# gabrieletiboni/random-envs

Hardware: AMD Instinct MI355X
Metric: env-steps/sec at batch 32768, RandomHopper-v0, 1/2/4/8 MI355X; % HBM roofline (higher is better)
Workload: dtype f32

## Files before the change

profiles/wavetime_probe.py:

```python
import os, sys, ctypes
os.environ.setdefault("REX_LIB", "librex_hip_wavetime.so")
sys.path.insert(0, os.path.dirname(os.path.dirname(os.path.abspath(__file__))))
import numpy as np, torch, random_envs_amd as rex
from random_envs_amd import _native
for eid in sys.argv[1:] or ["RandomHopper-v0"]:
    B = 32768
    env = rex.make(eid, batch=B, seed=0)
    nom = torch.tensor(env.original_task)
    env.set_dr_distribution("uniform", torch.stack([0.9 * nom, 1.1 * nom], 1).flatten().tolist()); env.set_dr_training(True); env.reset()
    g = torch.Generator().manual_seed(0)
    amp = 0.4 if "Humanoid" in eid else 1.0
    acts = [((torch.rand(env.dims.act_dim, B, generator=g) * 2 - 1) * amp).cuda() for _ in range(8)]
    for k in range(80 if "Humanoid" in eid else 300): env.step_soa(acts[k % 8])
    rows, infos = [], []
    info = (ctypes.c_ulonglong * (1024 * 8))(); torch.cuda.synchronize(); _native.lib().rex_debug_waveinfo(info, 1024)
    for k in range(20):
        env.step_soa(acts[k % 8]); torch.cuda.synchronize()
        out = (ctypes.c_ulonglong * 1024)(); _native.lib().rex_debug_wavetime(out, 1024)
        _native.lib().rex_debug_waveinfo(info, 1024)
        rows.append(np.array(list(out), dtype=np.float64)); infos.append(np.array(list(info), dtype=np.float64).reshape(1024, 8))
    w = np.stack(rows); I = np.stack(infos)
    if hasattr(_native.lib(), "rex_debug_wavephase") and "Humanoid" not in eid:
        ph = (ctypes.c_ulonglong * (1024 * 4))(); _native.lib().rex_debug_wavephase(ph, 1024)
        P = np.array(list(ph), dtype=np.float64).reshape(1024, 4)
        env.enable_timing(True); env.step_soa(acts[0]); torch.cuda.synchronize(); ms = env.read_timing()[-1]; env.enable_timing(False)
        print("   last launch, cycles per wave [mean / max]: load state %.0f / %.0f | substeps %.0f / %.0f | reward, obs, stores %.0f / %.0f | fused reset %.0f / %.0f | "
              "sum of means %.0f, slowest wave %.0f; kernel %.4f ms" % (P[:, 0].mean(), P[:, 0].max(), P[:, 1].mean(), P[:, 1].max(), P[:, 2].mean(), P[:, 2].max(),
                                                                     P[:, 3].mean(), P[:, 3].max(), P.sum(1).mean(), P.sum(1).max(), ms))
    if hasattr(_native.lib(), "rex_debug_evalphase") and "Humanoid" not in eid:
        ep = (ctypes.c_ulonglong * (1024 * 16))(); _native.lib().rex_debug_evalphase(ep, 1024)
        for k in range(10): env.step_soa(acts[k % 8])
        torch.cuda.synchronize(); _native.lib().rex_debug_evalphase(ep, 1024)
        E = np.array(list(ep), dtype=np.float64).reshape(1024, 16).mean(0) / 10
        nm = ["kinematics", "mass+bias+forces", "detect", "self / a0 / dispatch", "rows + solve", "  pass 1 (all)", "  pass 2 (all)"]
        print("   cycles per wave-step by phase of forward() (16 evaluations): " + " | ".join("%s %.0f" % (nm[k], E[k]) for k in range(7)) + " | sum of 0..4 %.0f" % E[:5].sum())
    print(eid, "cycles per wave-step: mean %.0f  p50 %.0f  p90 %.0f  p99 %.0f  max %.0f  -> max/mean %.2f" %
          (w.mean(), np.percentile(w, 50), np.percentile(w, 90), np.percentile(w, 99), w.max(1).mean(), w.max(1).mean() / w.mean()))
    print("   cycles in the fused reset path per wave-step: mean %.0f  p90 %.0f  max %.0f" % (I[..., 1].mean(), np.percentile(I[..., 1], 90), I[..., 1].max(1).mean()))
    print("   the same wave slow twice in a row (rank correlation of consecutive launches): %.2f" % np.corrcoef(w[:-1].ravel(), w[1:].ravel())[0, 1])
    names = ["solves", "reset cycles", "pass1", "pass2", "ls_evals", "nocon", "slots_active", "selfpath"]
    slow = w > np.percentile(w, 98); fast = w < np.percentile(w, 60)
    print("   per wave-step counts, typical waves (< p60) vs slow waves (> p98):")
    top = w.argmax(1)
    for k, nm in enumerate(names): print("     %-13s %8.1f %8.1f   slowest wave of each launch: mean %8.1f  min %8.1f  max %8.1f" %
                                         (nm, I[..., k][fast].mean(), I[..., k][slow].mean(), I[np.arange(len(top)), top, k].mean(), I[np.arange(len(top)), top, k].min(), I[np.arange(len(top)), top, k].max()))
    print("   per wave-step counts, mean over ALL waves: " + "  ".join("%s %.2f" % (nm, I[..., k].mean()) for k, nm in enumerate(names)))
    srt = np.sort(w, 1)
    print("   per launch: slowest wave %.0f, 2nd %.0f, 5th %.0f, 10th %.0f, 20th %.0f, 50th %.0f cycles (means over the launches)" %
          tuple(srt[:, -k].mean() for k in (1, 2, 5, 10, 20, 50)))
    env.close()
```

random-envs_amd/csrc/rex_hip.hip:

```cpp
#include <hip/hip_runtime.h>
#include <rocrand/rocrand_kernel.h>

#include <cmath>
#include <cstdarg>
#include <cstdio>
#include <cstdlib>
#include <cstring>
#include <new>
#include <vector>

#include "../../include/rex.h"
#include "planar_model.hpp"
#include "humanoid_model.hpp"
#include "humanoid_pair.hpp"

using namespace rex;

#ifdef REX_ONLY_KIND
#define REX_EN_CARTPOLE (REX_ONLY_KIND == 0)
#define REX_EN_HOPPER (REX_ONLY_KIND == 1)
#define REX_EN_HALFCHEETAH (REX_ONLY_KIND == 2)
#define REX_EN_WALKER2D (REX_ONLY_KIND == 3)
#define REX_EN_HUMANOID (REX_ONLY_KIND == 4)
#else
#define REX_EN_CARTPOLE 1
#define REX_EN_HOPPER 1
#define REX_EN_HALFCHEETAH 1
#define REX_EN_WALKER2D 1
#define REX_EN_HUMANOID 1
#endif

#if defined(REX_KTIME)
namespace rex { __device__ unsigned long long g_ktime[24 + 72]; }
extern "C" int rex_debug_ktime(unsigned long long* out) {
  if (hipMemcpyFromSymbol(out, HIP_SYMBOL(rex::g_ktime), sizeof(unsigned long long) * 96) != hipSuccess) return -1;
  unsigned long long z[96] = {0}; (void)hipMemcpyToSymbol(HIP_SYMBOL(rex::g_ktime), z, sizeof z); return 0; }
#endif
#if defined(REX_WAVETIME)
namespace rex { __device__ unsigned long long g_wavetime[8192]; __device__ unsigned long long g_waveinfo[8192][8]; __device__ unsigned long long g_wavehum[1024][16];
                __device__ unsigned long long g_wavephase[8192][4];
                __device__ unsigned long long g_waveplace[8192][4];
                }
#endif
#if defined(REX_WAVETIME) || defined(REX_PHASES)
namespace rex { __device__ unsigned long long g_evalphase[8192][16]; }
extern "C" int rex_debug_evalphase(unsigned long long* out, int n) {
  if (hipMemcpyFromSymbol(out, HIP_SYMBOL(rex::g_evalphase), sizeof(unsigned long long) * 16 * (n < 8192 ? n : 8192)) != hipSuccess) return -1;
  static unsigned long long z[8192][16]; return hipMemcpyToSymbol(HIP_SYMBOL(rex::g_evalphase), z, sizeof z) == hipSuccess ? 0 : -1; }
#endif
#if defined(REX_WAVETIME)
extern "C" int rex_debug_wavephase(unsigned long long* out, int n) {
  return hipMemcpyFromSymbol(out, HIP_SYMBOL(rex::g_wavephase), sizeof(unsigned long long) * 4 * (n < 8192 ? n : 8192)) == hipSuccess ? 0 : -1; }
extern "C" int rex_debug_waveplace(unsigned long long* out, int n) {
  return hipMemcpyFromSymbol(out, HIP_SYMBOL(rex::g_waveplace), sizeof(unsigned long long) * 4 * (n < 8192 ? n : 8192)) == hipSuccess ? 0 : -1; }
extern "C" int rex_debug_wavehum(unsigned long long* out) {
  return hipMemcpyFromSymbol(out, HIP_SYMBOL(rex::g_wavehum), sizeof(unsigned long long) * 1024 * 16) == hipSuccess ? 0 : -1; }
extern "C" int rex_debug_waveinfo(unsigned long long* out, int n) {
  if (hipMemcpyFromSymbol(out, HIP_SYMBOL(rex::g_waveinfo), sizeof(unsigned long long) * 8 * (n < 8192 ? n : 8192)) != hipSuccess) return -1;
  static unsigned long long z[8192][8]; return hipMemcpyToSymbol(HIP_SYMBOL(rex::g_waveinfo), z, sizeof z) == hipSuccess ? 0 : -1; }
extern "C" int rex_debug_wavetime(unsigned long long* out, int n) {
  return hipMemcpyFromSymbol(out, HIP_SYMBOL(rex::g_wavetime), sizeof(unsigned long long) * (n < 8192 ? n : 8192)) == hipSuccess ? 0 : -1; }
#endif
#if defined(REX_KSTATS)
namespace rex { __device__ unsigned long long g_kstats[8]; }
extern "C" int rex_debug_kstats(unsigned long long* out) {
  if (hipMemcpyFromSymbol(out, HIP_SYMBOL(rex::g_kstats), sizeof(unsigned long long) * 8) != hipSuccess) return -1;
  unsigned long long z[8] = {0}; (void)hipMemcpyToSymbol(HIP_SYMBOL(rex::g_kstats), z, sizeof z); return 0; }
#endif

static thread_local char g_err[512] = "";
static int set_err(int code, const char* fmt, ...) {
  va_list ap; va_start(ap, fmt); vsnprintf(g_err, sizeof g_err, fmt, ap); va_end(ap);
  return code;
}
#define HIP_TRY(x)                                                                            \
  do { hipError_t e_ = (x); if (e_ != hipSuccess) return set_err(REX_ERR_HIP, "%s failed: %s", #x, hipGetErrorString(e_)); } while (0)

extern "C" const char* rex_last_error(void) { return g_err; }
extern "C" const char* rex_version(void) { return "rex-hip 0.1 (gfx950)"; }

#define REX_ENTER(h, fn)                                                    \
  do { if (!(h)) return set_err(REX_ERR_ARG, fn ": null handle"); HIP_TRY(hipSetDevice((h)->device)); } while (0)

static const char* const kKnobs[] = {"REX_LANES", "REX_PAIR", "REX_ROLLED", "REX_HUM_PAIR", "REX_HUM_FUSED_RESET", "REX_FUSED_DERIVE",
                                     "REX_FAST", "REX_LS_MAX", "REX_LS_FREE", "REX_WARM", "REX_CORR",
                                     "REX_DIAG_NOCONTACT", "REX_HUM_ITERS"};
static bool tuning_allowed() { const char* e = getenv("REX_ALLOW_TUNING"); return e && atoi(e) == 1; }
static const char* stray_knob() {
  if (tuning_allowed()) return nullptr;
  for (const char* k : kKnobs) if (getenv(k)) return k;
  return nullptr;
}
static const char* knob(const char* name) { return tuning_allowed() ? getenv(name) : nullptr; }

constexpr int MAX_XI = 32;
struct DRParams {
  int type;
  int dim;
  float a[MAX_XI];
  float b[MAX_XI];
  float lower[MAX_XI];
  float lo[MAX_XI], hi[MAX_XI];
  int map[MAX_XI];
  const float* chol;
};

constexpr unsigned long long EP_STRIDE = 1ull << 32;
constexpr unsigned long long STEP_BASE = 512, STEP_STRIDE = 64;
constexpr unsigned long long SAMPLE_SEED_SALT = 0x9E3779B97F4A7C15ull;

__device__ __forceinline__ float truncnorm2(float u) {
  const float Fa = 0.022750131948179195f, Fb = 0.9772498680518208f;
  float p = Fa + u * (Fb - Fa);
  float x = normcdfinvf(p);
  return fminf(fmaxf(x, -2.0f), 2.0f);
}

__device__ void sample_task(const DRParams& dr, unsigned long long seed, unsigned long long subseq, unsigned long long offset,
                            float* __restrict__ xi_rows, size_t B, unsigned i, unsigned long long* counters) {
  const int d = dr.dim;
  rocrand_state_philox4x32_10 st;
  rocrand_init(seed, subseq, offset, &st);
  if (dr.type == REX_DR_UNIFORM) {
    for (int k = 0; k < d; k++) { float u = rocrand_uniform(&st); (xi_rows + (size_t)dr.map[k] * B)[i] = dr.a[k] + (dr.b[k] - dr.a[k]) * (1.0f - u); }
  } else if (dr.type == REX_DR_TRUNCNORM) {
    for (int k = 0; k < d; k++) {
      float lb = dr.lower[k];
      float obs = dr.a[k] + dr.b[k] * truncnorm2(rocrand_uniform(&st));
      for (int att = 0; att < 2 && obs < lb; att++) obs = dr.a[k] + dr.b[k] * truncnorm2(rocrand_uniform(&st));
      if (obs < lb) obs = lb;
      (xi_rows + (size_t)dr.map[k] * B)[i] = obs;
    }
  } else if (dr.type == REX_DR_GAUSSIAN) {
    for (int k = 0; k < d; k++) {
      float obs = dr.a[k] + dr.b[k] * rocrand_normal(&st);
      for (int att = 0; att < 2 && obs < 0.1f; att++) obs = dr.a[k] + dr.b[k] * rocrand_normal(&st);
      if (obs < 0.1f) { obs = 0.1f; atomicAdd(counters + 1, 1ull); }
      (xi_rows + (size_t)dr.map[k] * B)[i] = obs;
    }
  } else if (dr.type == REX_DR_FULLGAUSSIAN) {
    for (int k = 0; k < d; k++) {
      rocrand_state_philox4x32_10 sz; rocrand_init(seed, subseq, offset, &sz);
      float acc = dr.a[k];
      for (int j = 0; j <= k; j++) acc += dr.chol[k * MAX_XI + j] * rocrand_normal(&sz);
      acc = fminf(fmaxf(acc, 0.0f), 4.0f);
      (xi_rows + (size_t)dr.map[k] * B)[i] = acc * (dr.hi[k] - dr.lo[k]) * 0.25f + dr.lo[k];
    }
  }
}

struct DevState {
  float* qpos; float* qvel; float* xi;
  float* geom;
  float* aux;
  int* t; unsigned* episode; unsigned char* done;
  unsigned long long* counters;
  long long B, env_offset;
  unsigned long long seed;
};

struct StepFlags {
  int endless, noisy, time_limit, max_steps;
  float noise_std;
  float* info;
  int readonly;
};

__global__ void __launch_bounds__(64) cartpole_step_kernel(DevState s, StepFlags fl, const int* __restrict__ action,
                                                           float* __restrict__ obs, float* __restrict__ reward,
                                                           unsigned char* __restrict__ done_out, unsigned char* __restrict__ trunc_out,
                                                           float* __restrict__ term_obs) {
  const unsigned i = blockIdx.x * blockDim.x + threadIdx.x;
  if (i >= s.B) return;
  const long long B = s.B;
  float x = s.qpos[i], th = s.qpos[B + i], xd = s.qvel[i], thd = s.qvel[B + i];
  float g = s.xi[i], mc = s.xi[B + i], mp = s.xi[2 * B + i], l = s.xi[3 * B + i];
  float total = mp + mc;
  const float pml = 0.1f * 0.5f;
  float force = action[i] == 1 ? 10.0f : -10.0f;
  float st, ct; sincosf(th, &st, &ct);
  float temp = (force + pml * thd * thd * st) / total;
  float thacc = (g * st - ct * temp) / (l * (4.0f / 3.0f - mp * ct * ct / total));
  float xacc = temp - pml * thacc * ct / total;
  const float tau = 0.02f;
  x = x + tau * xd; xd = xd + tau * xacc; th = th + tau * thd; thd = thd + tau * thacc;
  s.qpos[i] = x; s.qpos[B + i] = th; s.qvel[i] = xd; s.qvel[B + i] = thd;
  const float th_thr = 12.0f * 2.0f * 3.14159265358979323846f / 360.0f, x_thr = 2.4f;
  bool was_done = s.done[i] != 0;
  bool dn = (x < -x_thr) || (x > x_thr) || (th < -th_thr) || (th > th_thr);
  float r = (!dn) ? 1.0f : (was_done ? 0.0f : 1.0f);
  int t = s.t[i] + 1; s.t[i] = t;
  bool trunc = fl.time_limit && t >= fl.max_steps && !dn;
  bool d = dn || trunc;
  s.done[i] = (unsigned char)((dn || was_done) ? 1 : 0) | (unsigned char)(d ? 2 : 0);
  obs[i] = x; obs[B + i] = xd; obs[2 * B + i] = th; obs[3 * B + i] = thd;
  if (term_obs) { term_obs[i] = x; term_obs[B + i] = xd; term_obs[2 * B + i] = th; term_obs[3 * B + i] = thd; }
  reward[i] = r; done_out[i] = d ? 1 : 0;
  if (trunc_out) trunc_out[i] = trunc ? 1 : 0;
}

__global__ void __launch_bounds__(64) cartpole_reset_kernel(DevState s, DRParams dr, int resample, int reset_state,
                                                            const unsigned char* __restrict__ mask, int mask_bit,
                                                            float* __restrict__ obs) {
  const unsigned i = blockIdx.x * blockDim.x + threadIdx.x;
  if (i >= s.B) return;
  if (mask && !(mask[i] & mask_bit)) return;
  const long long B = s.B;
  unsigned ep = s.episode[i] + 1; s.episode[i] = ep;
  rocrand_state_philox4x32_10 st;
  rocrand_init(s.seed, (unsigned long long)(s.env_offset + i), (unsigned long long)ep * EP_STRIDE, &st);
  if (reset_state) {
    float v[4];
#pragma unroll
    for (int k = 0; k < 4; k++) v[k] = -0.05f + 0.1f * (1.0f - rocrand_uniform(&st));
    s.qpos[i] = v[0]; s.qvel[i] = v[1]; s.qpos[B + i] = v[2]; s.qvel[B + i] = v[3];
    s.t[i] = 0; s.done[i] = 0;
    if (obs) { obs[i] = v[0]; obs[B + i] = v[1]; obs[2 * B + i] = v[2]; obs[3 * B + i] = v[3]; }
  }
  if (resample && dr.type != REX_DR_NONE) {
    sample_task(dr, s.seed, (unsigned long long)(s.env_offset + i), (unsigned long long)ep * EP_STRIDE + 256, s.xi, (size_t)B, i, s.counters);
  }
}

template <class S> constexpr int geom_floats() { return sizeof(PlanarGeom<float, S>) / sizeof(float); }

template <class S>
__device__ __forceinline__ void load_geom(const DevState& s, unsigned i, const PlanarGeom<float, S>& uniform,
                                          PlanarGeom<float, S>& G) {
  if constexpr (S::KIND == 3) {
    walker_expand(uniform, [&](int k) { return (s.geom + (size_t)k * s.B)[i]; }, G);
  } else {
    G = uniform;
  }
}

template <class S>
__device__ __forceinline__ void write_obs(const float (&q)[S::NV], const float (&v)[S::NV], float* __restrict__ obs,
                                          long long B, unsigned i, bool noisy, float noise_std,
                                          rocrand_state_philox4x32_10* st) {
  static_for<0, S::NOBS>([&](auto KK) {
    constexpr int k = KK;
    float o = k < S::NV - 1 ? q[k + 1] : v[k - (S::NV - 1)];
    if (noisy) o += noise_std * rocrand_normal(st);
    (obs + (size_t)k * B)[i] = o;
  });
}

template <class S>
__device__ __forceinline__ void planar_reset_lane(const DevState& s, const StepFlags& fl, const DRParams& dr, int resample,
                                                  int reset_state, unsigned i, float* __restrict__ obs);
__device__ __forceinline__ void walker_derive_lane(const DevState& s, unsigned i, int refresh_frozen_masses);
__device__ __attribute__((noinline)) void walker_derive_call(const DevState& s, unsigned i, int refresh_frozen_masses);
constexpr int RS_RESAMPLE = 1, RS_DERIVE = 2, RS_REFRESH = 4;

#ifndef REX_STEP_WAVES
#define REX_STEP_WAVES 1
#endif
#define REX_STEP_OCC __attribute__((amdgpu_waves_per_eu(REX_STEP_WAVES, REX_STEP_WAVES)))

template <class S, bool PAIR, bool ROLLED = false>
__global__ void __launch_bounds__(64) __attribute__((amdgpu_waves_per_eu(ROLLED ? 2 : REX_STEP_WAVES, ROLLED ? 2 : REX_STEP_WAVES)))
planar_step_kernel(DevState s, StepFlags fl, PlanarGeom<float, S> ugeom,
                                                         SolParams<float> sp, const float* __restrict__ action,
                                                         float* __restrict__ obs, float* __restrict__ reward,
                                                         unsigned char* __restrict__ done_out,
                                                         unsigned char* __restrict__ trunc_out, float* __restrict__ term_obs,
                                                         DRParams dr, int fused_reset, int resample) {
#if defined(REX_WAVETIME)
  const unsigned long long tp0 = __builtin_amdgcn_s_memtime();
  const unsigned long long tw0 = __builtin_amdgcn_s_memrealtime();
#endif
  unsigned blk = blockIdx.x;
  if constexpr (PAIR) { if (blockDim.x < 64u && (gridDim.x & 7u) == 0u) blk = (blk & 7u) * (gridDim.x >> 3) + (blk >> 3); }
  const unsigned i = (blk * blockDim.x + threadIdx.x) >> (PAIR ? 1 : 0);
  if (i >= s.B) return;
  const long long B = s.B;
  float q[S::NV], v[S::NV], ctrl[S::NU], xi[S::NXI];
  static_for<0, S::NV>([&](auto KK) { constexpr int k = KK; q[k] = (s.qpos + (size_t)k * B)[i]; v[k] = (s.qvel + (size_t)k * B)[i]; });
  static_for<0, S::NU>([&](auto KK) { constexpr int k = KK; ctrl[k] = (action + (size_t)k * B)[i]; });
  static_for<0, S::NXI>([&](auto KK) { constexpr int k = KK; xi[k] = (s.xi + (size_t)k * B)[i]; });
  PlanarGeom<float, S> G; load_geom<S>(s, i, ugeom, G);
  LaneParams<float, S> P; lane_params(S{}, xi, P);
#if defined(REX_KTIME) || defined(REX_WAVETIME)
  unsigned long long tk0 = __builtin_amdgcn_s_memtime();
#endif
  const float x_before = q[0];
  q[0] = 0.0f;
  bool capped = false;
  float acc[S::NV];
  static_for<0, S::NV>([&](auto KK) { acc[KK] = 0.0f; });
  constexpr int GEN = PAIR ? 2 : (ROLLED ? 1 : 0);
  float* slot_col = nullptr;
  if constexpr (GEN == 2) {
    __shared__ float slot_lds[SlotMem<float, S, PAIR>::WORDS];
    slot_col = slot_lds + threadIdx.x;
  }
#pragma unroll 1
  for (int f = 0; f < S::FRAME_SKIP; f++) capped |= substep<float, S, PAIR, GEN>(q, v, ctrl, G, P, sp, acc, f > 0, slot_col);
  if (PAIR && (threadIdx.x & 1u)) return;
  unsigned io = i; asm volatile("" : "+v"(io));
#if defined(REX_KTIME)
  if ((threadIdx.x & 63) == 0) atomicAdd(&g_ktime[5], __builtin_amdgcn_s_memtime() - tk0);
#endif
#if defined(REX_WAVETIME)
  const unsigned long long tk1 = __builtin_amdgcn_s_memtime();
  if ((threadIdx.x & 63) == 0) g_wavetime[blockIdx.x & 8191] = tk1 - tk0;
#endif
  const float dx = q[0];
  q[0] = x_before + dx;
  float asq = 0.0f;
  static_for<0, S::NU>([&](auto KK) { asq += ctrl[KK] * ctrl[KK]; });
  const float dt = float(S::TIMESTEP * S::FRAME_SKIP);
  float r = dx / dt + S::ALIVE - S::CTRL_COST * asq;
  bool finite = true;
  static_for<0, S::NV>([&](auto KK) { constexpr int k = KK; finite = finite && isfinite(q[k]) && isfinite(v[k]); });
  bool dn = false;
  if constexpr (S::KIND == 1) {
    bool small = true;
    static_for<2, S::NV>([&](auto KK) { constexpr int k = KK; small = small && fabsf(q[k]) < 100.0f; });
    static_for<0, S::NV>([&](auto KK) { constexpr int k = KK; small = small && fabsf(v[k]) < 100.0f; });
    dn = !(finite && small && q[1] > 0.7f && fabsf(q[2]) < 0.2f);
  } else if constexpr (S::KIND == 3) {
    dn = !(q[1] > 0.8f && q[1] < 2.0f && q[2] > -1.0f && q[2] < 1.0f);
  } else {
    dn = false;
  }
  if (fl.endless) dn = false;
  if (!fl.readonly) {
    if (!finite) atomicAdd(s.counters + 0, 1ull);
    if (capped && threadIdx.x == 0) atomicAdd(s.counters + 2, 1ull);
  }
  int t = s.t[io] + 1;
  bool trunc = fl.time_limit && t >= fl.max_steps && !dn && !fl.readonly;
  bool d = dn || trunc;
  if (!fl.readonly) {
    s.t[io] = t;
    static_for<0, S::NV>([&](auto KK) { constexpr int k = KK; (s.qpos + (size_t)k * B)[io] = q[k]; (s.qvel + (size_t)k * B)[io] = v[k]; });
    s.done[io] = d ? 2 : 0;
  }
  rocrand_state_philox4x32_10 st;
  if (fl.noisy) rocrand_init(s.seed, (unsigned long long)(s.env_offset + io),
                             (unsigned long long)s.episode[io] * EP_STRIDE + STEP_BASE + (unsigned long long)t * STEP_STRIDE, &st);
  write_obs<S>(q, v, obs, B, io, fl.noisy != 0, fl.noise_std, &st);
  if (term_obs) static_for<0, S::NOBS>([&](auto KK) { constexpr int k = KK; (term_obs + (size_t)k * B)[io] = (obs + (size_t)k * B)[io]; });
  reward[io] = r; done_out[io] = d ? 1 : 0;
  if (trunc_out) trunc_out[io] = trunc ? 1 : 0;
  if (fl.info) { fl.info[io] = dx / dt; (fl.info + (size_t)B)[io] = -S::CTRL_COST * asq; }
#if defined(REX_WAVETIME)
  const unsigned long long tr0 = __builtin_amdgcn_s_memtime();
#endif
  if (fused_reset && d) {
    planar_reset_lane<S>(s, fl, dr, resample & RS_RESAMPLE, 1, io, obs);
    if constexpr (S::KIND == 3) {
      if (resample & RS_DERIVE) {
        if constexpr (PAIR) walker_derive_lane(s, io, (resample & RS_REFRESH) ? 1 : 0);
        else walker_derive_call(s, io, (resample & RS_REFRESH) ? 1 : 0);
      }
    }
  }
#if defined(REX_WAVETIME)
  if ((threadIdx.x & 63) == 0) { g_waveinfo[blockIdx.x & 8191][1] += __builtin_amdgcn_s_memtime() - tr0; }
  if ((threadIdx.x & 63) == 0) { unsigned long long* ph = g_wavephase[blockIdx.x & 8191]; ph[0] = tk0 - tp0; ph[1] = tk1 - tk0; ph[2] = tr0 - tk1; ph[3] = __builtin_amdgcn_s_memtime() - tr0; }
  if ((threadIdx.x & 63) == 0) { unsigned long long* pl = g_waveplace[blockIdx.x & 8191]; pl[0] = tw0; pl[1] = __builtin_amdgcn_s_memrealtime();
    pl[2] = __builtin_amdgcn_s_getreg((31 << 11) | (0 << 6) | 4); pl[3] = __builtin_amdgcn_s_getreg((3 << 11) | (0 << 6) | 20); }
#endif
}

template <class S>
__device__ __forceinline__ void planar_reset_lane(const DevState& s, const StepFlags& fl, const DRParams& dr, int resample,
                                                  int reset_state, unsigned i, float* __restrict__ obs) {
  const long long B = s.B;
  unsigned ep = s.episode[i] + 1; s.episode[i] = ep;
#if defined(REX_DIAG_CHEAP_RESET)
  if (reset_state) {
    static_for<0, S::NV>([&](auto KK) { constexpr int k = KK; (s.qpos + (size_t)k * B)[i] = (k == 1 && S::KIND != 2) ? 1.25f : 0.0f; (s.qvel + (size_t)k * B)[i] = 0.0f; });
    s.t[i] = 0; s.done[i] = 0;
  }
  return;
#endif
  if (reset_state) {
    rocrand_state_philox4x32_10 st;
    rocrand_init(s.seed, (unsigned long long)(s.env_offset + i), (unsigned long long)ep * EP_STRIDE, &st);
    float q[S::NV], v[S::NV];
    const float c = S::INIT_NOISE;
    static_for<0, S::NV>([&](auto KK) { constexpr int k = KK;
      q[k] = c * (2.0f * (1.0f - rocrand_uniform(&st)) - 1.0f);
      if constexpr (S::KIND == 2) v[k] = 0.1f * rocrand_normal(&st);
      else v[k] = c * (2.0f * (1.0f - rocrand_uniform(&st)) - 1.0f);
    });
    if constexpr (S::KIND != 2) q[1] += 1.25f;
    static_for<0, S::NV>([&](auto KK) { constexpr int k = KK; (s.qpos + (size_t)k * B)[i] = q[k]; (s.qvel + (size_t)k * B)[i] = v[k]; });
    s.t[i] = 0; s.done[i] = 0;
    if (obs) {
      rocrand_state_philox4x32_10 st2;
      if (fl.noisy) rocrand_init(s.seed, (unsigned long long)(s.env_offset + i), (unsigned long long)ep * EP_STRIDE + STEP_BASE, &st2);
      write_obs<S>(q, v, obs, B, i, fl.noisy != 0, fl.noise_std, &st2);
    }
  }
  if (resample && dr.type != REX_DR_NONE) {
    sample_task(dr, s.seed, (unsigned long long)(s.env_offset + i), (unsigned long long)ep * EP_STRIDE + 256, s.xi, (size_t)B, i, s.counters);
  }
}

template <class S>
__global__ void __launch_bounds__(64) planar_reset_kernel(DevState s, StepFlags fl, DRParams dr, int resample, int reset_state,
                                                          const unsigned char* __restrict__ mask, int mask_bit,
                                                          float* __restrict__ obs, int pending_bit) {
  const unsigned i = blockIdx.x * blockDim.x + threadIdx.x;
  if (i >= s.B) return;
  if (mask && !(mask[i] & mask_bit)) return;
  planar_reset_lane<S>(s, fl, dr, resample, reset_state, i, obs);
  if (pending_bit) s.done[i] = (unsigned char)pending_bit;
}

#if REX_EN_WALKER2D
__global__ void __launch_bounds__(64) walker_derive_kernel(DevState s, const unsigned char* mask, int mask_bit,
                                                           int refresh_frozen_masses, int clear_pending) {
  using S = Walker2dSpec;
  const unsigned i = blockIdx.x * blockDim.x + threadIdx.x;
  if (i >= s.B) return;
  if (mask && !(mask[i] & mask_bit)) return;
  if (clear_pending) s.done[i] = 0;
  walker_derive_lane(s, i, refresh_frozen_masses);
}
__device__ __forceinline__ void walker_derive_lane(const DevState& s, unsigned i, int refresh_frozen_masses) {
  using S = Walker2dSpec;
  double size[4];
  for (int k = 0; k < 4; k++) size[k] = (double)s.xi[(long long)(7 + k) * s.B + i];
  PlanarGeom<double, S> G; SolParams<double> sp; double nominal[S::NB];
  derive_model<double, S>(size, G, nominal, sp);
  double c[kWalkerCompact];
  walker_compact_from_geom(G, c);
  for (int k = 0; k < kWalkerCompact; k++) (s.geom + (size_t)k * s.B)[i] = (float)c[k];
  if (refresh_frozen_masses) for (int b = 0; b < 3; b++) (s.xi + (size_t)b * s.B)[i] = (float)nominal[b];
}
__device__ __attribute__((noinline)) void walker_derive_call(const DevState& s, unsigned i, int refresh_frozen_masses) { walker_derive_lane(s, i, refresh_frozen_masses); }
#else
__device__ __forceinline__ void walker_derive_lane(const DevState&, unsigned, int) {}
__device__ __forceinline__ void walker_derive_call(const DevState&, unsigned, int) {}

#endif

template <class S>
__global__ void __launch_bounds__(64) planar_obs_kernel(DevState s, float* __restrict__ obs) {
  const unsigned i = blockIdx.x * blockDim.x + threadIdx.x;
  if (i >= s.B) return;
  float q[S::NV], v[S::NV];
  static_for<0, S::NV>([&](auto KK) { constexpr int k = KK; q[k] = (s.qpos + (size_t)k * s.B)[i]; v[k] = (s.qvel + (size_t)k * s.B)[i]; });
  write_obs<S>(q, v, obs, s.B, i, false, 0.0f, nullptr);
}
__global__ void __launch_bounds__(64) cartpole_obs_kernel(DevState s, float* __restrict__ obs) {
  const unsigned i = blockIdx.x * blockDim.x + threadIdx.x;
  if (i >= s.B) return;
  const long long B = s.B;
  obs[i] = s.qpos[i]; obs[B + i] = s.qvel[i]; obs[2 * B + i] = s.qpos[B + i]; obs[3 * B + i] = s.qvel[B + i];
}
__global__ void fill_rows_kernel(float* dst, const float* vals, int nrows, long long B) {
  long long i = (long long)blockIdx.x * blockDim.x + threadIdx.x;
  if (i >= B) return;
  for (int k = 0; k < nrows; k++) dst[(long long)k * B + i] = vals[k];
}

#if REX_EN_HUMANOID
__constant__ hum::Model<float> c_hum;

__device__ __forceinline__ void hum_lane(const DevState& s, unsigned i, hum::Lane<float>& L) {
  L.mass[0] = 0.0f;
  for (int k = 0; k < 13; k++) L.mass[1 + k] = (s.xi + (size_t)k * s.B)[i];
  for (int d = 0; d < 6; d++) L.damping[d] = 0.0f;
  for (int k = 0; k < 17; k++) L.damping[6 + k] = (s.xi + (size_t)(13 + k) * s.B)[i];
}

__global__ void __launch_bounds__(64) humanoid_step_kernel(DevState s, StepFlags fl, const float* __restrict__ action,
                                                           float* __restrict__ obs, float* __restrict__ reward,
                                                           unsigned char* __restrict__ done_out, unsigned char* __restrict__ trunc_out,
                                                           float* __restrict__ term_obs) {
  const unsigned i = blockIdx.x * blockDim.x + threadIdx.x;
  if (i >= s.B) return;
  const size_t B = (size_t)s.B;
  hum::Lane<float> L; hum_lane(s, i, L);
  float q[hum::NQ], v[hum::NV], a[hum::NU], xp[hum::NBODY];
  for (int k = 0; k < hum::NQ; k++) q[k] = (s.qpos + k * B)[i];
  for (int k = 0; k < hum::NV; k++) v[k] = (s.qvel + k * B)[i];
  for (int k = 0; k < hum::NU; k++) a[k] = (action + k * B)[i];
  for (int b = 0; b < hum::NBODY; b++) xp[b] = (s.aux + b * B)[i];
  hum::Kin<float> kn; hum::Scratch<float> sc;
#if defined(REX_KTIME)
  for (int k = 0; k < HT_SLOTS; k++) kn.tacc[k] = 0;
#endif
  float r; bool dn;
  rocrand_state_philox4x32_10 st;
  int t = s.t[i] + 1;
  if (fl.noisy) rocrand_init(s.seed, (unsigned long long)(s.env_offset + i),
                             (unsigned long long)s.episode[i] * EP_STRIDE + STEP_BASE + (unsigned long long)t * STEP_STRIDE, &st);
#if defined(REX_WAVETIME)
  const unsigned long long tk0 = __builtin_amdgcn_s_memtime();
#endif
  float terms[4];
  hum::env_step(c_hum, L, q, v, a, xp, kn, sc, r, dn, [&](int k, float val) {
    if (fl.noisy && k < 45) val += fl.noise_std * rocrand_normal(&st);
    (obs + k * B)[i] = val;
    if (term_obs) (term_obs + k * B)[i] = val;
  }, terms);
  if (fl.info) for (int k = 0; k < 4; k++) (fl.info + k * B)[i] = terms[k];
#if defined(REX_WAVETIME)
  if ((threadIdx.x & 63) == 0) g_wavetime[blockIdx.x & 8191] = __builtin_amdgcn_s_memtime() - tk0;
#endif
#if defined(REX_KTIME)
  for (int k = 0; k < HT_SLOTS; k++) {
    unsigned long long v = kn.tacc[k];
    for (int off = 32; off > 0; off >>= 1) { unsigned long long o = __shfl_xor(v, off); v = o > v ? o : v; }
    if ((threadIdx.x & 63) == 0) atomicAdd(&g_ktime[8 + k], v);
#if defined(REX_WAVETIME)
    if ((threadIdx.x & 63) == 0 && k < 16) g_wavehum[blockIdx.x & 1023][k] = v;
#endif
  }
#endif
  bool finite = true;
  for (int k = 0; k < hum::NQ; k++) finite = finite && isfinite(q[k]);
  for (int k = 0; k < hum::NV; k++) finite = finite && isfinite(v[k]);
  if (!finite) dn = true;
  if (fl.endless && finite) dn = false;
  bool trunc = fl.time_limit && t >= fl.max_steps && !dn && !fl.readonly;
  bool d = dn || trunc;
  if (!fl.readonly) {
    if (!finite) atomicAdd(s.counters + 0, 1ull);
    if (kn.overflow) atomicAdd(s.counters + 3, 1ull);
    s.t[i] = t;
    for (int k = 0; k < hum::NQ; k++) (s.qpos + k * B)[i] = q[k];
    for (int k = 0; k < hum::NV; k++) (s.qvel + k * B)[i] = v[k];
    for (int b = 0; b < hum::NBODY; b++) (s.aux + b * B)[i] = xp[b];
    s.done[i] = d ? 2 : 0;
  }
  reward[i] = r; done_out[i] = d ? 1 : 0;
  if (trunc_out) trunc_out[i] = trunc ? 1 : 0;
}

struct DevPair {
#if defined(__HIP_DEVICE_COMPILE__)
  __device__ __forceinline__ int side() const { return (int)(threadIdx.x & 1u); }
  __device__ __forceinline__ float xchg(float x) const { return pair_xchg(x); }
  __device__ __forceinline__ unsigned xchg(unsigned x) const { return pair_xchg(x); }
  __device__ __forceinline__ bool any(bool b) const { return REX_WAVE_ANY(b); }
  __device__ __forceinline__ float* col() const { return hum::hum_lds + (threadIdx.x >> 1) * hum::pr::PAIR_WORDS; }
  __device__ __forceinline__ void sync() const {
    __builtin_amdgcn_fence(__ATOMIC_RELEASE, "wavefront"); __builtin_amdgcn_wave_barrier(); __builtin_amdgcn_fence(__ATOMIC_ACQUIRE, "wavefront");
  }
#else
  __device__ int side() const { return 0; }
  __device__ float xchg(float x) const { return x; }
  __device__ unsigned xchg(unsigned x) const { return x; }
  __device__ bool any(bool b) const { return b; }
  __device__ float* col() const { return nullptr; }
  __device__ void sync() const {}
#endif
};

__global__ void __launch_bounds__(64) humanoid_pair_step_kernel(DevState s, StepFlags fl, const float* __restrict__ action,
                                                                float* __restrict__ obs, float* __restrict__ reward,
                                                                unsigned char* __restrict__ done_out, unsigned char* __restrict__ trunc_out,
                                                                float* __restrict__ term_obs, DRParams dr, int fused_reset, int resample) {
  namespace pr = hum::pr;
  const unsigned lane = blockIdx.x * blockDim.x + threadIdx.x;
  const unsigned i = lane >> 1;
  if (i >= s.B) return;
  const bool left = (lane & 1u) != 0u;
  const size_t B = (size_t)s.B;
  const DevPair p;
  pr::PLane<float> L;
  static_for<0, pr::LB>([&](auto BB) { constexpr int lb = BB; L.mass[lb] = (s.xi + (size_t)((left ? pr::gbL(lb) : pr::gbR(lb)) - 1) * B)[i]; });
  static_for<0, pr::LD>([&](auto DD) { constexpr int ld = DD;
    if constexpr (ld < 6) L.damping[ld] = 0.0f; else L.damping[ld] = (s.xi + (size_t)(13 + (left ? pr::gdL(ld) : pr::gdR(ld)) - 6) * B)[i]; });
  float ql[pr::LQ], vl[pr::LD], cl[pr::LU], xp[pr::LB];
  static_for<0, 7>([&](auto KK) { constexpr int k = KK; ql[k] = (s.qpos + (size_t)k * B)[i]; });
  static_for<6, pr::LD>([&](auto DD) { constexpr int ld = DD; ql[ld + 1] = (s.qpos + (size_t)((left ? pr::gdL(ld) : pr::gdR(ld)) + 1) * B)[i]; });
  static_for<0, pr::LD>([&](auto DD) { constexpr int ld = DD; vl[ld] = (s.qvel + (size_t)(left ? pr::gdL(ld) : pr::gdR(ld)) * B)[i]; });
  static_for<6, pr::LD>([&](auto DD) { constexpr int ld = DD;
    constexpr int uR = ld == 6 ? 1 : ld == 7 ? 0 : ld == 8 ? 2 : ld < 13 ? 3 + (ld - 9) : 11 + (ld - 13);
    constexpr int uL = ld < 9 ? uR : ld < 13 ? 7 + (ld - 9) : 14 + (ld - 13);
    cl[ld - 6] = (action + (size_t)(left ? uL : uR) * B)[i]; });
  static_for<0, pr::LB>([&](auto BB) { constexpr int lb = BB; xp[lb] = (s.aux + (size_t)(left ? pr::gbL(lb) : pr::gbR(lb)) * B)[i]; });
  float asq_side = 0.0f, asq = 0.0f;
  static_for<0, 3>([&](auto KK) { asq += cl[KK] * cl[KK]; });
  static_for<3, pr::LU>([&](auto KK) { asq_side += cl[KK] * cl[KK]; });
  asq += pr::psum(p, asq_side);
  pr::PKin<float> kn; pr::PScratch<float> sc; pr::PObs<float> park;
#if defined(REX_KTIME)
  for (int k = 0; k < HT_SLOTS; k++) kn.tacc[k] = 0;
#endif
  const int t = s.t[i] + 1;
#if defined(REX_WAVETIME)
  const unsigned long long tk0 = __builtin_amdgcn_s_memtime();
#endif
  float r, terms[4]; bool dn;
  pr::env_step(p, c_hum, L, ql, vl, cl, asq, xp, kn, sc, park, r, dn, terms);
#if defined(REX_WAVETIME)
  if ((threadIdx.x & 63) == 0) g_wavetime[blockIdx.x & 8191] = __builtin_amdgcn_s_memtime() - tk0;
#endif
#if defined(REX_KTIME)
  for (int k = 0; k < HT_SLOTS; k++) {
    unsigned long long v = kn.tacc[k];
    for (int off = 32; off > 0; off >>= 1) { unsigned long long o = __shfl_xor(v, off); v = o > v ? o : v; }
    if ((threadIdx.x & 63) == 0) atomicAdd(&g_ktime[8 + k], v);
#if defined(REX_WAVETIME)
    if ((threadIdx.x & 63) == 0 && k < 16) g_wavehum[blockIdx.x & 1023][k] = v;
#endif
  }
#endif
  float nz[45];
  if (fl.noisy) {
    rocrand_state_philox4x32_10 st;
    rocrand_init(s.seed, (unsigned long long)(s.env_offset + i), (unsigned long long)s.episode[i] * EP_STRIDE + STEP_BASE + (unsigned long long)t * STEP_STRIDE, &st);
    for (int k = 0; k < 45; k++) nz[k] = fl.noise_std * rocrand_normal(&st);
  }
  pr::emit_obs(p, ql, vl, park, [&](auto RR, auto RL, float val) {
    constexpr int rr = RR, rl = RL;
    if constexpr (rr < 45 && rl < 45) { if (fl.noisy) val += left ? nz[rl] : nz[rr]; }
    const size_t row = left ? (size_t)rl : (size_t)rr;
    (obs + row * B)[i] = val;
    if (term_obs) (term_obs + row * B)[i] = val;
  });
  bool finite = true;
  static_for<0, pr::LQ>([&](auto KK) { finite = finite && isfinite(ql[KK]); });
  static_for<0, pr::LD>([&](auto KK) { finite = finite && isfinite(vl[KK]); });
  finite = finite && (p.xchg(finite ? 1u : 0u) != 0u);
  if (!finite) dn = true;
  if (fl.endless && finite) dn = false;
  const bool trunc = fl.time_limit && t >= fl.max_steps && !dn && !fl.readonly;
  const bool d = dn || trunc;
  if (!fl.readonly) {
    static_for<9, pr::LD>([&](auto DD) { constexpr int ld = DD; const size_t g = left ? pr::gdL(ld) : pr::gdR(ld);
      (s.qpos + (g + 1) * B)[i] = ql[ld + 1]; (s.qvel + g * B)[i] = vl[ld]; });
    static_for<3, pr::LB>([&](auto BB) { constexpr int lb = BB; (s.aux + (size_t)(left ? pr::gbL(lb) : pr::gbR(lb)) * B)[i] = xp[lb]; });
  }
  if (!left) {
    if (!fl.readonly) {
      if (!finite) atomicAdd(s.counters + 0, 1ull);
      if (kn.overflow) atomicAdd(s.counters + 3, 1ull);
      s.t[i] = t;
      static_for<0, 10>([&](auto KK) { constexpr int k = KK; (s.qpos + (size_t)k * B)[i] = ql[k]; });
      static_for<0, 9>([&](auto KK) { constexpr int k = KK; (s.qvel + (size_t)k * B)[i] = vl[k]; });
      static_for<0, 3>([&](auto BB) { constexpr int lb = BB; (s.aux + (size_t)(lb + 1) * B)[i] = xp[lb]; });
      s.aux[i] = 0.0f;
      s.done[i] = d ? 2 : 0;
    }
    if (fl.info) for (int k = 0; k < 4; k++) (fl.info + k * B)[i] = terms[k];
    reward[i] = r; done_out[i] = d ? 1 : 0;
    if (trunc_out) trunc_out[i] = trunc ? 1 : 0;
  }
  if (fused_reset && d) {
    const unsigned ep = s.episode[i] + 1;
    rocrand_state_philox4x32_10 st;
    rocrand_init(s.seed, (unsigned long long)(s.env_offset + i), (unsigned long long)ep * EP_STRIDE, &st);
    static_for<0, hum::NQ>([&](auto KK) { constexpr int k = KK;
      const float val = c_hum.qpos0[k] + 0.01f * (2.0f * (1.0f - rocrand_uniform(&st)) - 1.0f);
      if constexpr (k < 10) ql[k] = val;
      else static_for<9, pr::LD>([&](auto DD) { constexpr int ld = DD;
        if constexpr (pr::gdR(ld) + 1 == k) ql[ld + 1] = left ? ql[ld + 1] : val;
        if constexpr (pr::gdL(ld) + 1 == k) ql[ld + 1] = left ? val : ql[ld + 1]; }); });
    static_for<0, hum::NV>([&](auto KK) { constexpr int k = KK;
      const float val = 0.01f * (2.0f * (1.0f - rocrand_uniform(&st)) - 1.0f);
      if constexpr (k < 9) vl[k] = val;
      else static_for<9, pr::LD>([&](auto DD) { constexpr int ld = DD;
        if constexpr (pr::gdR(ld) == k) vl[ld] = left ? vl[ld] : val;
        if constexpr (pr::gdL(ld) == k) vl[ld] = left ? val : vl[ld]; }); });
// ... 841 lines not shown
```

Baseline: 405.9 million.

## Inline fused reset in register epilogue with direct Philox blocks and prefetched t/episode

The step epilogue now computes observations and reset state in registers and writes qpos/qvel/t/done/obs once. Before, it stored the stepped state and obs and then overwrote them in the reset path. The Philox counters for observation noise, reset noise and uniform DR sampling are generated directly as whole blocks instead of through rocrand state init. t and episode are loaded at kernel start and parked in shared memory, so their global loads are off the tail. The aim is to shorten the tail latency of waves that hit resets. The risks are that the RNG streams must stay bit-identical to rocrand's and that the shared parking assumes 64-thread blocks.

```diff
diff --git a/profiles/wavetime_probe.py b/profiles/wavetime_probe.py
--- a/profiles/wavetime_probe.py
+++ b/profiles/wavetime_probe.py
@@ -27,6 +27,20 @@
         print("   last launch, cycles per wave [mean / max]: load state %.0f / %.0f | substeps %.0f / %.0f | reward, obs, stores %.0f / %.0f | fused reset %.0f / %.0f | "
               "sum of means %.0f, slowest wave %.0f; kernel %.4f ms" % (P[:, 0].mean(), P[:, 0].max(), P[:, 1].mean(), P[:, 1].max(), P[:, 2].mean(), P[:, 2].max(),
                                                                      P[:, 3].mean(), P[:, 3].max(), P.sum(1).mean(), P.sum(1).max(), ms))
+    if hasattr(_native.lib(), "rex_debug_wavetail") and "Humanoid" not in eid:
+        tl = (ctypes.c_ulonglong * (1024 * 8))(); _native.lib().rex_debug_wavetail(tl, 1024)
+        env.step_soa(acts[1]); torch.cuda.synchronize()
+        _native.lib().rex_debug_wavephase(ph, 1024); _native.lib().rex_debug_wavetail(tl, 1024)
+        P = np.array(list(ph), dtype=np.float64).reshape(1024, 4); T = np.array(list(tl), dtype=np.float64).reshape(1024, 8)
+        rs = T[:, 5] > 0
+        seg = [("t returned", T[:, 0]), ("reward logic, stepped stores issued", T[:, 1] - T[:, 0])]
+        if rs.any():
+            R = T[rs]
+            seg += [("episode returned", R[:, 2]), ("state draws + stores", R[:, 3] - R[:, 2]), ("xi draws + stores", R[:, 4] - R[:, 3]),
+                    ("rest of the reset (walker2d: re-derive)", R[:, 5] - R[:, 4])]
+        print("   tail of one launch, cycles per wave [mean / max] (%d of %d waves ran the reset; reset rows over those): " % (rs.sum(), len(rs)) +
+              " | ".join("%s %.0f / %.0f" % (nm, x.mean(), x.max()) for nm, x in seg) +
+              " | whole tail (load state + epilogue + reset) %.0f / %.0f" % ((P[:, 0] + P[:, 2] + P[:, 3]).mean(), (P[:, 0] + P[:, 2] + P[:, 3]).max()))
     if hasattr(_native.lib(), "rex_debug_evalphase") and "Humanoid" not in eid:
         ep = (ctypes.c_ulonglong * (1024 * 16))(); _native.lib().rex_debug_evalphase(ep, 1024)
         for k in range(10): env.step_soa(acts[k % 8])
diff --git a/random-envs_amd/csrc/rex_hip.hip b/random-envs_amd/csrc/rex_hip.hip
--- a/random-envs_amd/csrc/rex_hip.hip
+++ b/random-envs_amd/csrc/rex_hip.hip
@@ -39,6 +39,7 @@
 #if defined(REX_WAVETIME)
 namespace rex { __device__ unsigned long long g_wavetime[8192]; __device__ unsigned long long g_waveinfo[8192][8]; __device__ unsigned long long g_wavehum[1024][16];
                 __device__ unsigned long long g_wavephase[8192][4];
+                __device__ unsigned long long g_wavetail[8192][8];
                 __device__ unsigned long long g_waveplace[8192][4];
                 }
 #endif
@@ -51,6 +52,9 @@
 #if defined(REX_WAVETIME)
 extern "C" int rex_debug_wavephase(unsigned long long* out, int n) {
   return hipMemcpyFromSymbol(out, HIP_SYMBOL(rex::g_wavephase), sizeof(unsigned long long) * 4 * (n < 8192 ? n : 8192)) == hipSuccess ? 0 : -1; }
+extern "C" int rex_debug_wavetail(unsigned long long* out, int n) {
+  if (hipMemcpyFromSymbol(out, HIP_SYMBOL(rex::g_wavetail), sizeof(unsigned long long) * 8 * (n < 8192 ? n : 8192)) != hipSuccess) return -1;
+  static unsigned long long z[8192][8]; return hipMemcpyToSymbol(HIP_SYMBOL(rex::g_wavetail), z, sizeof z) == hipSuccess ? 0 : -1; }
 extern "C" int rex_debug_waveplace(unsigned long long* out, int n) {
   return hipMemcpyFromSymbol(out, HIP_SYMBOL(rex::g_waveplace), sizeof(unsigned long long) * 4 * (n < 8192 ? n : 8192)) == hipSuccess ? 0 : -1; }
 extern "C" int rex_debug_wavehum(unsigned long long* out) {
@@ -116,37 +120,95 @@
   return fminf(fmaxf(x, -2.0f), 2.0f);
 }
 
+struct EngineRng {
+  rocrand_state_philox4x32_10 st;
+  __device__ __forceinline__ EngineRng(unsigned long long seed, unsigned long long subseq, unsigned long long offset) { rocrand_init(seed, subseq, offset, &st); }
+  __device__ __forceinline__ float uniform() { return rocrand_uniform(&st); }
+  __device__ __forceinline__ float normal() { return rocrand_normal(&st); }
+};
+template <class RNG = EngineRng>
 __device__ void sample_task(const DRParams& dr, unsigned long long seed, unsigned long long subseq, unsigned long long offset,
                             float* __restrict__ xi_rows, size_t B, unsigned i, unsigned long long* counters) {
   const int d = dr.dim;
-  rocrand_state_philox4x32_10 st;
-  rocrand_init(seed, subseq, offset, &st);
+  RNG st(seed, subseq, offset);
   if (dr.type == REX_DR_UNIFORM) {
-    for (int k = 0; k < d; k++) { float u = rocrand_uniform(&st); (xi_rows + (size_t)dr.map[k] * B)[i] = dr.a[k] + (dr.b[k] - dr.a[k]) * (1.0f - u); }
+    for (int k = 0; k < d; k++) { float u = st.uniform(); (xi_rows + (size_t)dr.map[k] * B)[i] = dr.a[k] + (dr.b[k] - dr.a[k]) * (1.0f - u); }
   } else if (dr.type == REX_DR_TRUNCNORM) {
     for (int k = 0; k < d; k++) {
       float lb = dr.lower[k];
-      float obs = dr.a[k] + dr.b[k] * truncnorm2(rocrand_uniform(&st));
-      for (int att = 0; att < 2 && obs < lb; att++) obs = dr.a[k] + dr.b[k] * truncnorm2(rocrand_uniform(&st));
+      float obs = dr.a[k] + dr.b[k] * truncnorm2(st.uniform());
+      for (int att = 0; att < 2 && obs < lb; att++) obs = dr.a[k] + dr.b[k] * truncnorm2(st.uniform());
       if (obs < lb) obs = lb;
       (xi_rows + (size_t)dr.map[k] * B)[i] = obs;
     }
   } else if (dr.type == REX_DR_GAUSSIAN) {
     for (int k = 0; k < d; k++) {
-      float obs = dr.a[k] + dr.b[k] * rocrand_normal(&st);
-      for (int att = 0; att < 2 && obs < 0.1f; att++) obs = dr.a[k] + dr.b[k] * rocrand_normal(&st);
+      float obs = dr.a[k] + dr.b[k] * st.normal();
+      for (int att = 0; att < 2 && obs < 0.1f; att++) obs = dr.a[k] + dr.b[k] * st.normal();
       if (obs < 0.1f) { obs = 0.1f; atomicAdd(counters + 1, 1ull); }
       (xi_rows + (size_t)dr.map[k] * B)[i] = obs;
     }
   } else if (dr.type == REX_DR_FULLGAUSSIAN) {
     for (int k = 0; k < d; k++) {
-      rocrand_state_philox4x32_10 sz; rocrand_init(seed, subseq, offset, &sz);
+      RNG sz(seed, subseq, offset);
       float acc = dr.a[k];
-      for (int j = 0; j <= k; j++) acc += dr.chol[k * MAX_XI + j] * rocrand_normal(&sz);
+      for (int j = 0; j <= k; j++) acc += dr.chol[k * MAX_XI + j] * sz.normal();
       acc = fminf(fmaxf(acc, 0.0f), 4.0f);
       (xi_rows + (size_t)dr.map[k] * B)[i] = acc * (dr.hi[k] - dr.lo[k]) * 0.25f + dr.lo[k];
     }
   }
+}
+
+__device__ __forceinline__ void philox_block(unsigned long long seed, unsigned long long subseq, unsigned long long block, unsigned* __restrict__ w) {
+  unsigned c0 = (unsigned)block, c1 = (unsigned)(block >> 32), c2 = (unsigned)subseq, c3 = (unsigned)(subseq >> 32);
+  unsigned k0 = (unsigned)seed, k1 = (unsigned)(seed >> 32);
+#pragma unroll
+  for (int r = 0; r < 10; r++) {
+    const unsigned hi0 = __umulhi(0xD2511F53u, c0), lo0 = 0xD2511F53u * c0;
+    const unsigned hi1 = __umulhi(0xCD9E8D57u, c2), lo1 = 0xCD9E8D57u * c2;
+    c0 = hi1 ^ c1 ^ k0; c1 = lo1; c2 = hi0 ^ c3 ^ k1; c3 = lo0;
+    k0 += 0x9E3779B9u; k1 += 0xBB67AE85u;
+  }
+  w[0] = c0; w[1] = c1; w[2] = c2; w[3] = c3;
+}
+template <int NBLK>
+__device__ __forceinline__ void philox_blocks(unsigned long long seed, unsigned long long subseq, unsigned long long block0, unsigned (&w)[4 * NBLK]) {
+  static_for<0, NBLK>([&](auto BB) { constexpr int b = BB; philox_block(seed, subseq, block0 + (unsigned long long)b, w + 4 * b); });
+}
+__device__ __forceinline__ float philox_uniform(unsigned w) { return rocrand_device::detail::uniform_distribution(w); }
+__device__ __forceinline__ float2 philox_normal2(unsigned w0, unsigned w1) { return rocrand_device::detail::normal_distribution2(w0, w1); }
+
+struct PhiloxWords {
+  unsigned long long seed, subseq, block; unsigned w[4]; int n; float saved; bool has;
+  __device__ __forceinline__ PhiloxWords(unsigned long long seed_, unsigned long long subseq_, unsigned long long offset)
+      : seed(seed_), subseq(subseq_), block(offset >> 2), n(4), saved(0.0f), has(false) {}
+  __device__ __forceinline__ unsigned next() {
+    if (n == 4) { philox_block(seed, subseq, block, w); block++; n = 0; }
+    const unsigned r = n == 0 ? w[0] : n == 1 ? w[1] : n == 2 ? w[2] : w[3];
+    n++;
+    return r;
+  }
+  __device__ __forceinline__ float uniform() { return philox_uniform(next()); }
+  __device__ __forceinline__ float normal() {
+    if (has) { has = false; return saved; }
+    const unsigned a = next(), b = next();
+    const float2 r = philox_normal2(a, b);
+    saved = r.y; has = true;
+    return r.x;
+  }
+};
+
+template <int NXI>
+__device__ __forceinline__ void sample_task_uniform(const DRParams& dr, unsigned long long seed, unsigned long long subseq, unsigned long long offset,
+                                                    float* __restrict__ xi_rows, size_t B, unsigned i) {
+  const int d = dr.dim;
+  float a[NXI], b[NXI]; int m[NXI];
+  static_for<0, NXI>([&](auto KK) { constexpr int k = KK; a[k] = dr.a[k]; b[k] = dr.b[k]; m[k] = dr.map[k]; });
+  constexpr int NBLK = (NXI + 3) / 4;
+  unsigned w[4 * NBLK];
+  static_for<0, NBLK>([&](auto BB) { constexpr int bb = BB; if (4 * bb < d) philox_block(seed, subseq, (offset >> 2) + (unsigned long long)bb, w + 4 * bb); });
+  static_for<0, NXI>([&](auto KK) { constexpr int k = KK;
+    if (k < d) { float u = philox_uniform(w[k]); (xi_rows + (size_t)m[k] * B)[i] = a[k] + (b[k] - a[k]) * (1.0f - u); } });
 }
 
 struct DevState {
@@ -247,6 +309,40 @@
 }
 
 template <class S>
+__device__ __forceinline__ void obs_values(const float (&q)[S::NV], const float (&v)[S::NV], float (&ob)[S::NOBS], bool noisy, float noise_std,
+                                           unsigned long long seed, unsigned long long subseq, unsigned long long offset) {
+  static_for<0, S::NOBS>([&](auto KK) { constexpr int k = KK; ob[k] = k < S::NV - 1 ? q[k + 1] : v[k - (S::NV - 1)]; });
+  if (noisy) {
+    constexpr int NP = (S::NOBS + 1) / 2, NBLK = (2 * NP + 3) / 4;
+    unsigned w[4 * NBLK];
+    philox_blocks<NBLK>(seed, subseq, offset >> 2, w);
+    static_for<0, NP>([&](auto PP) { constexpr int p = PP;
+      const float2 n = philox_normal2(w[2 * p], w[2 * p + 1]);
+      ob[2 * p] += noise_std * n.x;
+      if constexpr (2 * p + 1 < S::NOBS) ob[2 * p + 1] += noise_std * n.y; });
+  }
+}
+template <class S>
+__device__ __forceinline__ void reset_state_values(unsigned long long seed, unsigned long long subseq, unsigned ep, float (&q)[S::NV], float (&v)[S::NV]) {
+  constexpr int NV = S::NV;
+  constexpr int NW = S::KIND == 2 ? 4 * (NV / 2) + (NV % 2 ? 3 : 0) : 2 * NV, NBLK = (NW + 3) / 4;
+  unsigned w[4 * NBLK];
+  philox_blocks<NBLK>(seed, subseq, ((unsigned long long)ep * EP_STRIDE) >> 2, w);
+  const float c = S::INIT_NOISE;
+  if constexpr (S::KIND == 2) {
+    static_for<0, (NV + 1) / 2>([&](auto PP) { constexpr int p = PP;
+      const float2 n = philox_normal2(w[4 * p + 1], w[4 * p + 2]);
+      q[2 * p] = c * (2.0f * (1.0f - philox_uniform(w[4 * p])) - 1.0f); v[2 * p] = 0.1f * n.x;
+      if constexpr (2 * p + 1 < NV) { q[2 * p + 1] = c * (2.0f * (1.0f - philox_uniform(w[4 * p + 3])) - 1.0f); v[2 * p + 1] = 0.1f * n.y; } });
+  } else {
+    static_for<0, NV>([&](auto KK) { constexpr int k = KK;
+      q[k] = c * (2.0f * (1.0f - philox_uniform(w[2 * k])) - 1.0f);
+      v[k] = c * (2.0f * (1.0f - philox_uniform(w[2 * k + 1])) - 1.0f); });
+    q[1] += 1.25f;
+  }
+}
+
+template <class S>
 __device__ __forceinline__ void planar_reset_lane(const DevState& s, const StepFlags& fl, const DRParams& dr, int resample,
                                                   int reset_state, unsigned i, float* __restrict__ obs);
 __device__ __forceinline__ void walker_derive_lane(const DevState& s, unsigned i, int refresh_frozen_masses);
@@ -275,10 +371,13 @@
   const unsigned i = (blk * blockDim.x + threadIdx.x) >> (PAIR ? 1 : 0);
   if (i >= s.B) return;
   const long long B = s.B;
+  __shared__ unsigned tail_park[2 * 64];
+  const int t_in = s.t[i]; const unsigned ep_in = s.episode[i];
   float q[S::NV], v[S::NV], ctrl[S::NU], xi[S::NXI];
   static_for<0, S::NV>([&](auto KK) { constexpr int k = KK; q[k] = (s.qpos + (size_t)k * B)[i]; v[k] = (s.qvel + (size_t)k * B)[i]; });
   static_for<0, S::NU>([&](auto KK) { constexpr int k = KK; ctrl[k] = (action + (size_t)k * B)[i]; });
   static_for<0, S::NXI>([&](auto KK) { constexpr int k = KK; xi[k] = (s.xi + (size_t)k * B)[i]; });
+  tail_park[threadIdx.x] = (unsigned)t_in; tail_park[64 + threadIdx.x] = ep_in;
   PlanarGeom<float, S> G; load_geom<S>(s, i, ugeom, G);
   LaneParams<float, S> P; lane_params(S{}, xi, P);
 #if defined(REX_KTIME) || defined(REX_WAVETIME)
@@ -330,37 +429,69 @@
     if (!finite) atomicAdd(s.counters + 0, 1ull);
     if (capped && threadIdx.x == 0) atomicAdd(s.counters + 2, 1ull);
   }
-  int t = s.t[io] + 1;
+  unsigned lo = threadIdx.x; asm volatile("" : "+v"(lo));
+  const unsigned ep_prev = tail_park[64 + lo];
+  int t = (int)tail_park[lo] + 1;
+#if defined(REX_WAVETIME)
+  asm volatile("s_waitcnt lgkmcnt(0)" ::: "memory"); const unsigned long long tt0 = __builtin_amdgcn_s_memtime();
+#endif
   bool trunc = fl.time_limit && t >= fl.max_steps && !dn && !fl.readonly;
   bool d = dn || trunc;
-  if (!fl.readonly) {
-    s.t[io] = t;
-    static_for<0, S::NV>([&](auto KK) { constexpr int k = KK; (s.qpos + (size_t)k * B)[io] = q[k]; (s.qvel + (size_t)k * B)[io] = v[k]; });
-    s.done[io] = d ? 2 : 0;
-  }
-  rocrand_state_philox4x32_10 st;
-  if (fl.noisy) rocrand_init(s.seed, (unsigned long long)(s.env_offset + io),
-                             (unsigned long long)s.episode[io] * EP_STRIDE + STEP_BASE + (unsigned long long)t * STEP_STRIDE, &st);
-  write_obs<S>(q, v, obs, B, io, fl.noisy != 0, fl.noise_std, &st);
-  if (term_obs) static_for<0, S::NOBS>([&](auto KK) { constexpr int k = KK; (term_obs + (size_t)k * B)[io] = (obs + (size_t)k * B)[io]; });
+  const unsigned long long subseq = (unsigned long long)(s.env_offset + io);
+  float ob[S::NOBS];
+  obs_values<S>(q, v, ob, fl.noisy != 0, fl.noise_std, s.seed, subseq,
+                (unsigned long long)ep_prev * EP_STRIDE + STEP_BASE + (unsigned long long)t * STEP_STRIDE);
+  if (term_obs) static_for<0, S::NOBS>([&](auto KK) { constexpr int k = KK; (term_obs + (size_t)k * B)[io] = ob[k]; });
   reward[io] = r; done_out[io] = d ? 1 : 0;
   if (trunc_out) trunc_out[io] = trunc ? 1 : 0;
   if (fl.info) { fl.info[io] = dx / dt; (fl.info + (size_t)B)[io] = -S::CTRL_COST * asq; }
 #if defined(REX_WAVETIME)
   const unsigned long long tr0 = __builtin_amdgcn_s_memtime();
 #endif
+  unsigned char dflag = d ? 2 : 0;
   if (fused_reset && d) {
-    planar_reset_lane<S>(s, fl, dr, resample & RS_RESAMPLE, 1, io, obs);
+    const unsigned ep = ep_prev + 1; s.episode[io] = ep;
+#if defined(REX_WAVETIME)
+    atomicMax(&g_wavetail[blockIdx.x & 8191][2], __builtin_amdgcn_s_memtime() - tr0);
+#endif
+#if defined(REX_DIAG_CHEAP_RESET)
+    static_for<0, S::NV>([&](auto KK) { constexpr int k = KK; q[k] = (k == 1 && S::KIND != 2) ? 1.25f : 0.0f; v[k] = 0.0f; });
+    t = 0; dflag = 0;
+#else
+    reset_state_values<S>(s.seed, subseq, ep, q, v);
+    t = 0; dflag = 0;
+    obs_values<S>(q, v, ob, fl.noisy != 0, fl.noise_std, s.seed, subseq, (unsigned long long)ep * EP_STRIDE + STEP_BASE);
+#if defined(REX_WAVETIME)
+    atomicMax(&g_wavetail[blockIdx.x & 8191][3], __builtin_amdgcn_s_memtime() - tr0);
+#endif
+    if ((resample & RS_RESAMPLE) && dr.type != REX_DR_NONE) {
+      if (dr.type == REX_DR_UNIFORM && dr.dim <= S::NXI) sample_task_uniform<S::NXI>(dr, s.seed, subseq, (unsigned long long)ep * EP_STRIDE + 256, s.xi, (size_t)B, io);
+      else sample_task<PhiloxWords>(dr, s.seed, subseq, (unsigned long long)ep * EP_STRIDE + 256, s.xi, (size_t)B, io, s.counters);
+    }
+#if defined(REX_WAVETIME)
+    atomicMax(&g_wavetail[blockIdx.x & 8191][4], __builtin_amdgcn_s_memtime() - tr0);
+#endif
     if constexpr (S::KIND == 3) {
       if (resample & RS_DERIVE) {
         if constexpr (PAIR) walker_derive_lane(s, io, (resample & RS_REFRESH) ? 1 : 0);
         else walker_derive_call(s, io, (resample & RS_REFRESH) ? 1 : 0);
       }
     }
-  }
+#endif
+#if defined(REX_WAVETIME)
+    atomicMax(&g_wavetail[blockIdx.x & 8191][5], __builtin_amdgcn_s_memtime() - tr0);
+#endif
+  }
+  if (!fl.readonly) {
+    s.t[io] = t;
+    static_for<0, S::NV>([&](auto KK) { constexpr int k = KK; (s.qpos + (size_t)k * B)[io] = q[k]; (s.qvel + (size_t)k * B)[io] = v[k]; });
+    s.done[io] = dflag;
+  }
+  static_for<0, S::NOBS>([&](auto KK) { constexpr int k = KK; (obs + (size_t)k * B)[io] = ob[k]; });
 #if defined(REX_WAVETIME)
   if ((threadIdx.x & 63) == 0) { g_waveinfo[blockIdx.x & 8191][1] += __builtin_amdgcn_s_memtime() - tr0; }
   if ((threadIdx.x & 63) == 0) { unsigned long long* ph = g_wavephase[blockIdx.x & 8191]; ph[0] = tk0 - tp0; ph[1] = tk1 - tk0; ph[2] = tr0 - tk1; ph[3] = __builtin_amdgcn_s_memtime() - tr0; }
+  if ((threadIdx.x & 63) == 0) { unsigned long long* tl = g_wavetail[blockIdx.x & 8191]; tl[0] = tt0 - tk1; tl[1] = tr0 - tk1; }
   if ((threadIdx.x & 63) == 0) { unsigned long long* pl = g_waveplace[blockIdx.x & 8191]; pl[0] = tw0; pl[1] = __builtin_amdgcn_s_memrealtime();
     pl[2] = __builtin_amdgcn_s_getreg((31 << 11) | (0 << 6) | 4); pl[3] = __builtin_amdgcn_s_getreg((3 << 11) | (0 << 6) | 20); }
 #endif
```

Result: faster. 424.5 million, median of 6 (+4.6%).
